# LiZhuoHong/SegLand

Hardware: AMD Instinct MI355X
Metric: 512x512 tiles/sec fwd+bwd PSPNet-POP (higher is better)
Workload: dtype bf16; 1 GPU; PSPNet-POP resnet50 bf16, batch 16/GPU, 512x512, 8 logit channels, train_base.py loop body (fwd+loss+bwd+clip+AdamW x2), 1 x MI355X; global_batch=16, parallelism=dp1

## Files before the change

include/segland_hip_debug.h:

```cpp
#ifndef SEGLAND_HIP_DEBUG_H
#define SEGLAND_HIP_DEBUG_H
#include "segland_hip.h"
#ifdef __cplusplus
extern "C" {
#endif

void sl_debug_reset(void);

void sl_debug_conv_affine(int on);
void sl_debug_conv_p9(int on);
void sl_debug_conv_p8_k1(int on);
void sl_debug_conv_ring192(int on);
void sl_debug_conv_ringn64(int on);
void sl_debug_conv_rows_small(int on);
void sl_debug_ppm_fact_walk(int on);
void sl_debug_conv_parity(int on);
void sl_debug_ring_small_k(int k);
void sl_debug_ring64_max_tiles(int tiles);
void sl_debug_wgrad3(int on);
void sl_debug_wgrad_bias(int on);
void sl_debug_wgrad_tr(int on);
void sl_debug_wgrad_pair_min(int rows);
void sl_debug_attn_valu(int v);

void sl_debug_p8_trace(void* buf);
void sl_debug_wgrad_trace(void* buf);
void sl_debug_wgrad3_trace(void* buf);
void sl_debug_attn_trace(void* buf);

int sl_debug_wgrad3_plan(const SlConvDesc* d, int* out);

#ifdef __cplusplus
}
#endif
#endif
```

segland_amd/csrc/api.cpp:

```cpp
#include <stdarg.h>
#include <stdio.h>
#include "common.h"

static thread_local char g_err[512] = "";

void sl_set_error(const char* fmt, ...) {
  va_list ap;
  va_start(ap, fmt);
  vsnprintf(g_err, sizeof(g_err), fmt, ap);
  va_end(ap);
}

extern "C" int sl_version(void) { return 100; }
extern "C" const char* sl_last_error_string(void) { return g_err; }
extern "C" int sl_hip_clear_error(void) { return (int)hipGetLastError(); }

#include "../../include/segland_hip_debug.h"
SlDebugState g_sl_debug;
extern "C" void sl_debug_reset(void) { g_sl_debug = SlDebugState(); }
extern "C" void sl_debug_conv_affine(int v) { g_sl_debug.conv_affine = v ? 1 : 0; }
extern "C" void sl_debug_conv_p9(int v) { g_sl_debug.conv_p9 = (v & 1) ? 1 : 0; }
extern "C" void sl_debug_conv_p8_k1(int v) { g_sl_debug.conv_p8_k1 = v ? 1 : 0; }
extern "C" void sl_debug_conv_ring192(int v) { g_sl_debug.conv_ring192 = v ? 1 : 0; }
extern "C" void sl_debug_conv_ringn64(int v) { g_sl_debug.conv_ringn64 = v ? 1 : 0; }
extern "C" void sl_debug_conv_rows_small(int v) { g_sl_debug.conv_rows_small = v ? 1 : 0; }
extern "C" void sl_debug_conv_parity(int v) { g_sl_debug.conv_parity = v ? 1 : 0; }
extern "C" void sl_debug_ppm_fact_walk(int v) { g_sl_debug.ppm_fact_walk = v ? 1 : 0; }
extern "C" void sl_debug_ring64_max_tiles(int v) { g_sl_debug.ring64_max_tiles = v; }
extern "C" void sl_debug_ring_small_k(int v) { g_sl_debug.ring_small_k = v; }
extern "C" void sl_debug_wgrad3(int v) { g_sl_debug.wgrad3 = v ? 1 : 0; }
extern "C" void sl_debug_wgrad_bias(int v) { g_sl_debug.wgrad_bias = v ? 1 : 0; }
extern "C" void sl_debug_wgrad_tr(int v) { g_sl_debug.wgrad_tr = v ? 1 : 0; }
extern "C" void sl_debug_wgrad_pair_min(int rows) { g_sl_debug.wgrad_pair_min_rows = rows; }
extern "C" void sl_debug_attn_valu(int v) { g_sl_debug.attn_valu = v; }
extern "C" void sl_debug_p8_trace(void* buf) { g_sl_debug.p8_trace = (unsigned long long*)buf; }
extern "C" void sl_debug_wgrad_trace(void* buf) { g_sl_debug.wgrad_trace = (unsigned long long*)buf; }
extern "C" void sl_debug_wgrad3_trace(void* buf) { g_sl_debug.wgrad3_trace = (unsigned long long*)buf; }
extern "C" void sl_debug_attn_trace(void* buf) { g_sl_debug.attn_trace = (unsigned long long*)buf; }
```

segland_amd/csrc/common.h:

```cpp
#pragma once
#include <hip/hip_runtime.h>
#include <stdint.h>
#include <stdio.h>
#include "../../include/segland_hip.h"

typedef unsigned short bf16_t;

typedef __attribute__((ext_vector_type(8))) __bf16 bf16x8_t;
typedef __attribute__((ext_vector_type(16))) float f32x16_t;
typedef __attribute__((ext_vector_type(4))) float f32x4_t;

__device__ __forceinline__ float bf2f(bf16_t v) { return __uint_as_float(((unsigned)v) << 16); }
__device__ __forceinline__ bf16_t f2bf(float f) {
  return __builtin_bit_cast(bf16_t, (__bf16)f);
}

template <typename T> __device__ __forceinline__ float to_f(T v);
template <> __device__ __forceinline__ float to_f<float>(float v) { return v; }
template <> __device__ __forceinline__ float to_f<bf16_t>(bf16_t v) { return bf2f(v); }
template <typename T> __device__ __forceinline__ T from_f(float v);
template <> __device__ __forceinline__ float from_f<float>(float v) { return v; }
template <> __device__ __forceinline__ bf16_t from_f<bf16_t>(float v) { return f2bf(v); }

template <typename T> struct Vec16 { static constexpr int N = 16 / sizeof(T); };

template <typename T> __device__ __forceinline__ void unpack16(const uint4& v, float* out);
template <> __device__ __forceinline__ void unpack16<float>(const uint4& v, float* out) {
  out[0] = __uint_as_float(v.x); out[1] = __uint_as_float(v.y); out[2] = __uint_as_float(v.z); out[3] = __uint_as_float(v.w);
}
template <> __device__ __forceinline__ void unpack16<bf16_t>(const uint4& v, float* out) {
  out[0] = __uint_as_float(v.x << 16); out[1] = __uint_as_float(v.x & 0xffff0000u);
  out[2] = __uint_as_float(v.y << 16); out[3] = __uint_as_float(v.y & 0xffff0000u);
  out[4] = __uint_as_float(v.z << 16); out[5] = __uint_as_float(v.z & 0xffff0000u);
  out[6] = __uint_as_float(v.w << 16); out[7] = __uint_as_float(v.w & 0xffff0000u);
}
template <typename T> __device__ __forceinline__ uint4 pack16(const float* in);
template <> __device__ __forceinline__ uint4 pack16<float>(const float* in) {
  return make_uint4(__float_as_uint(in[0]), __float_as_uint(in[1]), __float_as_uint(in[2]), __float_as_uint(in[3]));
}
template <> __device__ __forceinline__ uint4 pack16<bf16_t>(const float* in) {
  typedef __attribute__((ext_vector_type(2))) __bf16 bf16x2_t;
  typedef __attribute__((ext_vector_type(2))) float f32x2_t;
  uint4 r;
  r.x = __builtin_bit_cast(unsigned, __builtin_convertvector((f32x2_t){in[0], in[1]}, bf16x2_t));
  r.y = __builtin_bit_cast(unsigned, __builtin_convertvector((f32x2_t){in[2], in[3]}, bf16x2_t));
  r.z = __builtin_bit_cast(unsigned, __builtin_convertvector((f32x2_t){in[4], in[5]}, bf16x2_t));
  r.w = __builtin_bit_cast(unsigned, __builtin_convertvector((f32x2_t){in[6], in[7]}, bf16x2_t));
  return r;
}

__device__ __forceinline__ float sl_erf_as(float x) {
  const float ax = fabsf(x);
  const float t = __builtin_amdgcn_rcpf(fmaf(0.3275911f, ax, 1.f));
  float p = fmaf(1.061405429f, t, -1.453152027f);
  p = fmaf(p, t, 1.421413741f); p = fmaf(p, t, -0.284496736f); p = fmaf(p, t, 0.254829592f);
  const float r = fmaf(-p * t, __expf(-ax * ax), 1.f);
  return copysignf(r, x);
}
template <typename T> __device__ __forceinline__ float sl_gelu(float x) {
  if constexpr (sizeof(T) == 4) return 0.5f * x * (1.f + erff(x * 0.70710678118654752440f));
  else return 0.5f * x * (1.f + sl_erf_as(x * 0.70710678118654752440f));
}

template <typename T> __device__ __forceinline__ float sl_gelu_grad(float x) {
  const float pdf = 0.39894228040143267794f * __expf(-0.5f * x * x);
  float cdf;
  if constexpr (sizeof(T) == 4) cdf = 0.5f * (1.f + erff(x * 0.70710678118654752440f));
  else cdf = 0.5f * (1.f + sl_erf_as(x * 0.70710678118654752440f));
  return cdf + x * pdf;
}

__device__ __forceinline__ float wave_sum(float v) {
#pragma unroll
  for (int o = 32; o > 0; o >>= 1) v += __shfl_xor(v, o, 64);
  return v;
}

void sl_set_error(const char* fmt, ...);

struct SlDebugState {
  int conv_affine = 1;
  int conv_p9 = 1;
  int conv_p8_k1 = 1;
  int conv_ring192 = 1;
  int conv_ringn64 = 1;
  int conv_rows_small = 1;
  int ppm_fact_walk = 1;
  int conv_parity = 1;
  int ring_small_k = 128;
  long long ring64_max_tiles = 256;
  int wgrad3 = 1;
  int wgrad_bias = 1;
  int wgrad_tr = 1;
  long long wgrad_pair_min_rows = 0;
  int attn_valu = -1;
  unsigned long long* p8_trace = nullptr;
  unsigned long long* wgrad_trace = nullptr;
  unsigned long long* wgrad3_trace = nullptr;
  unsigned long long* attn_trace = nullptr;
};
extern SlDebugState g_sl_debug;
#define SL_REQUIRE(cond, ...)            \
  do {                                   \
    if (!(cond)) {                       \
      sl_set_error(__VA_ARGS__);         \
      return SL_EINVAL;                  \
    }                                    \
  } while (0)
#define SL_LAUNCH_CHECK(name)                                                \
  do {                                                                       \
    hipError_t e__ = hipGetLastError();                                      \
    if (e__ != hipSuccess) {                                                 \
      sl_set_error("%s: %s", name, hipGetErrorString(e__));                  \
      return (int)e__;                                                       \
    }                                                                        \
  } while (0)

__host__ __device__ static inline int cdiv(long long a, long long b) { return (int)((a + b - 1) / b); }

template <typename T>
__device__ __forceinline__ void sl_colsum_rows_block(const T* __restrict__ x, long long rows, int C, long long rows_per_block, float* __restrict__ part, int block, float* red) {
  constexpr int V = Vec16<T>::N;
  const int nvec = C / V;
  const int tpr = nvec < 256 ? nvec : 256, rpb = 256 / tpr;
  const int tr = threadIdx.x / tpr, tc = threadIdx.x % tpr;
  const long long r0 = (long long)block * rows_per_block, r1 = r0 + rows_per_block < rows ? r0 + rows_per_block : rows;
  for (int vc = tc; vc < nvec; vc += tpr) {
    float s[V];
#pragma unroll
    for (int k = 0; k < V; ++k) s[k] = 0.f;
    if (tr < rpb) {
      long long r = r0 + tr;
      for (; r + 3 * rpb < r1; r += 4 * rpb) {
        uint4 q[4];
#pragma unroll
        for (int u = 0; u < 4; ++u) q[u] = ((const uint4*)x)[(size_t)(r + u * rpb) * nvec + vc];
#pragma unroll
        for (int u = 0; u < 4; ++u) {
          float v[V];
          unpack16<T>(q[u], v);
#pragma unroll
          for (int k = 0; k < V; ++k) s[k] += v[k];
        }
      }
      for (; r < r1; r += rpb) {
        float v[V];
        unpack16<T>(((const uint4*)x)[(size_t)r * nvec + vc], v);
#pragma unroll
        for (int k = 0; k < V; ++k) s[k] += v[k];
      }
    }
    __syncthreads();
#pragma unroll
    for (int k = 0; k < V; ++k) red[threadIdx.x * V + k] = s[k];
    __syncthreads();
    if (tr == 0) {
#pragma unroll
      for (int k = 0; k < V; ++k) {
        float a = 0.f;
        for (int j = 0; j < rpb; ++j) a += red[(j * tpr + tc) * V + k];
        part[(size_t)block * C + vc * V + k] = a;
      }
    }
  }
}


inline long long sl_colsum_rows_chunk(long long rows, int C, int esize) {
  const int nvec = C * esize / 16, tpr = nvec < 256 ? nvec : 256, rpb = 256 / tpr;
  long long rpblk = (long long)rpb * 16;
  const long long cap = 2048;
  if ((rows + rpblk - 1) / rpblk > cap) rpblk = ((rows + cap - 1) / cap + rpb - 1) / rpb * rpb;
  return rpblk;
}
```

segland_amd/csrc/conv_gemm_common.h:

```cpp
#pragma once
#include <stdlib.h>
#include "common.h"

#ifndef SL_CH3_SPLIT
#define SL_CH3_SPLIT 2
#endif


struct ConvGemmParams {
  const void* src1; const void* src2;
  int C1, C2;
  const void* wt;
  void* out;
  int B, Hs, Ws;
  int Hd, Wd;
  int N, KH, KW, stride, pad, dil;
  int mode;
  const float* scale;
  const float* bias; int relu;
  const void* addend; const void* mask_src;
  const void* pre_addend;
  const unsigned char* addend_mask;
  float* stat_partial;
  const unsigned char* gate;
// ... 472 lines not shown
        for (int u = 0; u < CH; ++u) {
          const int m = mrow(it0 + u);
          if (m < p.M) prev[u] = *(const uint4*)((const T*)p.pre_addend + (size_t)m * p.N + ncol);
        }
      }
      unsigned abit[CH];
      if (p.addend) {
#pragma unroll
        for (int u = 0; u < CH; ++u) {
          const int m = mrow(it0 + u);
          if (m < p.M) addv[u] = *(const uint4*)((const T*)p.addend + (size_t)m * p.N + ncol);
        }
        if (p.addend_mask) {
#pragma unroll
          for (int u = 0; u < CH; ++u) {
            const int m = mrow(it0 + u);
            if (m < p.M) abit[u] = p.addend_mask[((size_t)m * p.N + ncol) / EPC];
          }
        }
      }
      if (p.mask_src) {
#pragma unroll
        for (int u = 0; u < CH; ++u) {
          const int m = mrow(it0 + u);
          if (m < p.M) mskv[u] = *(const uint4*)((const T*)p.mask_src + (size_t)m * p.N + ncol);
        }
      }
#pragma unroll
      for (int u = 0; u < CH; ++u) {
        const int row = r0 + (it0 + u) * RS;
        const int m = mrow(it0 + u);
        if (m < p.M) {
          float v[EPC];
          const uint4 raw = *(const uint4*)(smem + row * G::PITCH + cc * 16);
          unpack16<T>(raw, v);
          if (p.pre_addend) {
            float a[EPC];
            unpack16<T>(prev[u], a);
#pragma unroll
            for (int e = 0; e < EPC; ++e) v[e] += a[e];
          }
#pragma unroll
          for (int e = 0; e < EPC; ++e) { ssum[e] += v[e]; ssq[e] += v[e] * v[e]; }
          if (plain) { st16(out + (size_t)m * p.N + ncol, raw); continue; }
          if (p.bias || p.scale) {
#pragma unroll
            for (int e = 0; e < EPC; ++e) v[e] = v[e] * scl[e] + bias[e];
          }
          if (p.out2) {
            float g[EPC];
            unpack16<T>(pack16<T>(v), g);
#pragma unroll
            for (int e = 0; e < EPC; ++e) g[e] = sl_gelu<T>(g[e]);
            st16((T*)p.out2 + (size_t)m * p.N + ncol, pack16<T>(g));
          }
          if (p.row_scale) {
            const float rs = p.row_scale[m / (p.Hd * p.Wd)];
#pragma unroll
            for (int e = 0; e < EPC; ++e) v[e] *= rs;
          }
          if (p.addend) {
            float a[EPC];
            unpack16<T>(addv[u], a);
            if (p.addend_mask) {
              const unsigned bits = abit[u];
#pragma unroll
              for (int e = 0; e < EPC; ++e) a[e] = (bits >> e) & 1u ? a[e] : 0.f;
            }
#pragma unroll
            for (int e = 0; e < EPC; ++e) v[e] += a[e];
          }
          if (p.relu) {
#pragma unroll
            for (int e = 0; e < EPC; ++e) v[e] = v[e] > 0.f ? v[e] : 0.f;
          }
          if (p.mask_src) {
            float k[EPC];
            unpack16<T>(mskv[u], k);
            bool gelu = false;
            if constexpr (!SPLIT) gelu = (p.flags & 4) != 0;
            if (gelu) {
#pragma unroll
              for (int e = 0; e < EPC; ++e) v[e] *= sl_gelu_grad<T>(k[e]);
            } else {
#pragma unroll
              for (int e = 0; e < EPC; ++e) v[e] = k[e] > 0.f ? v[e] : 0.f;
            }
          }
          st16(out + (size_t)m * p.N + ncol, pack16<T>(v));
        }
      }
    }
    lds_barrier();
  }
  if (p.stat_partial) {
#pragma unroll
    for (int off = CPR; off < 64; off <<= 1) {
#pragma unroll
      for (int e = 0; e < EPC; ++e) { ssum[e] += __shfl_xor(ssum[e], off, 64); ssq[e] += __shfl_xor(ssq[e], off, 64); }
    }
    float* red = (float*)smem;
    const int wave = tid >> 6;
    if (lane < CPR) {
#pragma unroll
      for (int e = 0; e < EPC; ++e) {
        red[(wave * 2 + 0) * BN + cc * EPC + e] = ssum[e];
        red[(wave * 2 + 1) * BN + cc * EPC + e] = ssq[e];
      }
    }
    lds_barrier();
    for (int e = tid; e < 2 * BN; e += NT) {
      const int which = e / BN, col = e % BN;
      float t = 0.f;
#pragma unroll
      for (int w = 0; w < WM * WN; ++w) t += red[(w * 2 + which) * BN + col];
      p.stat_partial[((size_t)bm * 2 + which) * p.N + bn * BN + col] = t;
    }
  }
}

__device__ __attribute__((aligned(256))) unsigned char g_zero_page[256];

typedef __attribute__((address_space(3))) void lds_void_t;
typedef const __attribute__((address_space(1))) void gbl_void_t;

__device__ __forceinline__ void glds16(const void* g, unsigned char* l) {
  __builtin_amdgcn_global_load_lds((gbl_void_t*)g, (lds_void_t*)l, 16, 0, 0);
}

template <int RBYTES> __device__ __forceinline__ int ring_off(int row, int chunk);
template <> __device__ __forceinline__ int ring_off<128>(int row, int chunk) { return row * 128 + ((chunk ^ ((row >> 1) & 7)) << 4); }
template <> __device__ __forceinline__ int ring_off<64>(int row, int chunk) { return row * 64 + ((chunk ^ ((row >> 2) & 3)) << 4); }
template <int RBYTES> __device__ __forceinline__ int ring_swz(int row);
template <> __device__ __forceinline__ int ring_swz<128>(int row) { return (row >> 1) & 7; }
template <> __device__ __forceinline__ int ring_swz<64>(int row) { return (row >> 2) & 3; }

__device__ __forceinline__ void glds16_asm(const void* g, unsigned lds_addr) {
  unsigned keep;
  asm volatile("s_mov_b32 %0, m0\n\ts_mov_b32 m0, %2\n\ts_nop 0\n\tglobal_load_lds_dwordx4 %1, off\n\ts_mov_b32 m0, %0"
               : "=&s"(keep) : "v"(g), "s"(lds_addr) : "memory");
}
__device__ __forceinline__ void glds16x2_asm(const void* g0, const void* g1, unsigned lds_addr) {
  unsigned keep;
  asm volatile("s_mov_b32 %0, m0\n\ts_mov_b32 m0, %3\n\ts_nop 0\n\tglobal_load_lds_dwordx4 %1, off\n\ts_add_u32 m0, m0, 0x400\n\ts_nop 0\n\t"
               "global_load_lds_dwordx4 %2, off\n\ts_mov_b32 m0, %0"
               : "=&s"(keep) : "v"(g0), "v"(g1), "s"(lds_addr) : "memory", "scc");
}
__device__ __forceinline__ void glds16x2_sbase_asm(const void* sbase, unsigned off0, unsigned off1, unsigned lds_addr) {
  unsigned keep;
  asm volatile("s_mov_b32 %0, m0\n\ts_mov_b32 m0, %4\n\ts_nop 0\n\tglobal_load_lds_dwordx4 %2, %1\n\ts_add_u32 m0, m0, 0x400\n\ts_nop 0\n\t"
               "global_load_lds_dwordx4 %3, %1\n\ts_mov_b32 m0, %0"
               : "=&s"(keep) : "s"(sbase), "v"(off0), "v"(off1), "s"(lds_addr) : "memory", "scc");
}
__device__ __forceinline__ unsigned lds_addr_of(const unsigned char* p) {
  return (unsigned)(size_t)((const __attribute__((address_space(3))) unsigned char*)p);
}

template <int N> __device__ __forceinline__ void wait_vmcnt() { asm volatile("s_waitcnt vmcnt(%0)" ::"n"(N) : "memory"); }


}
```

segland_amd/csrc/conv_gemm_patch.hip:

```cpp
#include "conv_gemm_common.h"

namespace {

__device__ __forceinline__ void conv_store_partial(const ConvGemmParams& p, f32x16_t (&acc)[4][2], int part, int bm, int bn, int wm, int wn, int lane) {
  const int l31 = lane & 31, fh = lane >> 5;
  float* base = p.ws + (size_t)part * p.M * p.N + bn * 256 + wn * 32 + 4 * fh;
  int tbase = 0;
  if (p.tile16) { const int tx = p.Wd >> 4, ty = p.Hd >> 4; tbase = ((bm / (tx * ty)) * p.Hd + ((bm / tx) % ty) * 16) * p.Wd + (bm % tx) * 16; }
#pragma unroll
  for (int i = 0; i < 4; ++i) {
    const int R = (i >> 1) * 128 + wm * 64 + (i & 1) * 32 + l31;
    const int m = p.tile16 ? tbase + (R >> 4) * p.Wd + (R & 15) : bm * 256 + R;
    if (m < p.M) {
      float* row = base + (size_t)m * p.N;
#pragma unroll
      for (int j = 0; j < 2; ++j)
#pragma unroll
        for (int q = 0; q < 4; ++q)
          *(float4*)(row + j * 128 + 8 * q) = make_float4(acc[i][j][4 * q + 0], acc[i][j][4 * q + 1], acc[i][j][4 * q + 2], acc[i][j][4 * q + 3]);
    }
  }
}

template <typename T>
// ... 174 lines not shown

  int bm, bn;
  tile_of(blockIdx.x, bm, bn);
  setup(bm, bn);
  issue_first();
  int younger = 0;
  const bool counted = p.flags & 1;
#pragma unroll 1
  for (int tile = blockIdx.x; tile < ntiles; tile += gridDim.x) {
    f32x16_t acc[4][2];
#pragma unroll
    for (int i = 0; i < 4; ++i)
#pragma unroll
      for (int j = 0; j < 2; ++j)
#pragma unroll
        for (int r = 0; r < 16; ++r) acc[i][j][r] = 0.f;

    int tap2 = 0, ct2 = 0;
    adv(tap2, ct2);
    if (nk > 1) {
      issueB(0, tap2, ct2, p8_slot_b0(1)); issueA(0, tap2, ct2, p8_slot_a0(1)); issueA(1, tap2, ct2, p8_slot_a1(1)); issueB(1, tap2, ct2, p8_slot_b1(1));
      switch (younger) { case 16: wait_vmcnt<24>(); break; case 17: wait_vmcnt<25>(); break; case 32: wait_vmcnt<40>(); break; case 48: wait_vmcnt<56>(); break; case 49: wait_vmcnt<57>(); break; default: wait_vmcnt<8>(); }
    } else wait_vmcnt<0>();
    adv(tap2, ct2);
    __builtin_amdgcn_s_barrier();
    if (p.trace && tile == (int)blockIdx.x) tr1 = __builtin_amdgcn_s_memtime();
    uint4 a[4][2], b0k[4], b1k[4];
#pragma unroll
    for (int ks = 0; ks < 4; ++ks) { a[ks][0] = ldA(p8_slot_a0(0), 0, ks); a[ks][1] = ldA(p8_slot_a0(0), 1, ks); b0k[ks] = ldB(p8_slot_b0(0), ks); }

    int s3 = 0;
    if constexpr (!K1) {
    for (int i = 0; i < nk; ++i) {
      const int par = i & 1;
      const int s3n = s3 == 2 ? 0 : s3 + 1, s3nn = s3 == 0 ? 2 : s3 - 1;
      const int b0nxt = p8_slot_b0(s3n), b0nn = p8_slot_b0(s3nn);
      const int a1cur = p8_slot_a1(par), b1cur = p8_slot_b1(par), a0nxt = p8_slot_a0(s3n), a0nn = p8_slot_a0(s3nn);
      const bool more2 = i + 2 < nk;
#pragma unroll
      for (int q = 0; q < 16; ++q) {
        const int ph = q >> 2, ks = q & 3;
        const int ih = ph >> 1, jh = (ph == 1 || ph == 2) ? 1 : 0;
        if ((ks == 0 || ks == 2) && more2 && (ks == 2) == (wm == 1)) {
          if (ph == 0) issueB(0, tap2, ct2, b0nn);
          if (ph == 1) issueA(0, tap2, ct2, a0nn);
          if (ph == 3) { issueA(1, tap2, ct2, a1cur); issueB(1, tap2, ct2, b1cur); }
        }
        if (ph == 0) b1k[ks] = ldB(b1cur, ks);
        const uint4 bq = (ph == 0 || ph == 3) ? b0k[ks] : b1k[ks];
        Mma<T>::run(bq, a[ks][0], acc[ih * 2 + 0][jh]);
        Mma<T>::run(bq, a[ks][1], acc[ih * 2 + 1][jh]);
        if (ph == 1) { a[ks][0] = ldA(a1cur, 0, ks); a[ks][1] = ldA(a1cur, 1, ks); }
        if (ph == 3) { a[ks][0] = ldA(a0nxt, 0, ks); a[ks][1] = ldA(a0nxt, 1, ks); b0k[ks] = ldB(b0nxt, ks); }
        if (ks == 3) {
          if (ph == 2) { if (more2) wait_vmcnt<8>(); else if (i + 1 < nk) wait_vmcnt<4>(); else wait_vmcnt<0>(); }
          if (ph == 3) { if (more2) wait_vmcnt<8>(); else wait_vmcnt<0>(); }
          if (ph >= 2) __builtin_amdgcn_s_barrier();
        }
      }
      adv(tap2, ct2);
      s3 = s3 == 2 ? 0 : s3 + 1;
    }
    } else {
      auto ktile = [&](int i, auto tail_c) {
        constexpr int TAIL = decltype(tail_c)::value;
        const int par = i & 1;
        const int s3n = s3 == 2 ? 0 : s3 + 1, s3nn = s3 == 0 ? 2 : s3 - 1;
        const int b0nxt = p8_slot_b0(s3n), b0nn = p8_slot_b0(s3nn);
        const int a1cur = p8_slot_a1(par), b1cur = p8_slot_b1(par), a0nxt = p8_slot_a0(s3n), a0nn = p8_slot_a0(s3nn);
#pragma unroll
        for (int q = 0; q < 16; ++q) {
          const int ph = q >> 2, ks = q & 3;
          const int ih = ph >> 1, jh = (ph == 1 || ph == 2) ? 1 : 0;
          if (TAIL == 0 && (ks == 0 || ks == 2) && (ks == 2) == (wm == 1)) {
            if (ph == 0) issueB(0, 0, 0, b0nn);
            if (ph == 1) issueA(0, 0, 0, a0nn);
            if (ph == 3) { issueA(1, 0, 0, a1cur); issueB(1, 0, 0, b1cur); }
          }
          if (ph == 0) b1k[ks] = ldB(b1cur, ks);
          const uint4 bq = (ph == 0 || ph == 3) ? b0k[ks] : b1k[ks];
          Mma<T>::run(bq, a[ks][0], acc[ih * 2 + 0][jh]);
          Mma<T>::run(bq, a[ks][1], acc[ih * 2 + 1][jh]);
          if (ph == 1) { a[ks][0] = ldA(a1cur, 0, ks); a[ks][1] = ldA(a1cur, 1, ks); }
          if (ph == 3) { a[ks][0] = ldA(a0nxt, 0, ks); a[ks][1] = ldA(a0nxt, 1, ks); b0k[ks] = ldB(b0nxt, ks); }
          if (ks == 3) {
            if (ph == 2) wait_vmcnt<TAIL == 0 ? 8 : TAIL == 1 ? 4 : 0>();
            if (ph == 3) wait_vmcnt<TAIL == 0 ? 8 : 0>();
            if (ph >= 2) __builtin_amdgcn_s_barrier();
          }
        }
        s3 = s3 == 2 ? 0 : s3 + 1;
      };
      int i = 0;
#pragma unroll 1
      for (; i + 2 < nk; ++i) ktile(i, std::integral_constant<int, 0>());
      if (nk > 1) { ktile(i, std::integral_constant<int, 1>()); ++i; }
      ktile(i, std::integral_constant<int, 2>());
    }
    if (p.trace && tile == (int)blockIdx.x) tr2 = __builtin_amdgcn_s_memtime();
    lds_barrier();
    const int cbm = bm, cbn = bn;
    if (tile + (int)gridDim.x < ntiles) {
      tile_of(tile + gridDim.x, bm, bn);
      setup(bm, bn);
      issue_first();
    }
    younger = conv_epilogue_lds<T, BM, BN, 2, 4, true, GATE, AFF>(p, acc, cbm, cbn, wm, wn, lane, tid, smem);
    if (!counted) younger = 0;
    lds_barrier();
  }
  if (p.trace && tid == 0) {
    unsigned long long* t = p.trace + (size_t)blockIdx.x * 8;
    t[0] = tr0; t[1] = tr1; t[2] = tr2; t[3] = __builtin_amdgcn_s_memtime(); t[4] = __builtin_amdgcn_s_getreg((4 << 0) | (0 << 6) | (31 << 11)); t[5] = __builtin_amdgcn_s_getreg((20 << 0) | (0 << 6) | (31 << 11));
  }
}

int launch_splitk_finish(ConvGemmParams& p, hipStream_t st) {
  const size_t nvec = (size_t)p.M * p.N / 8;
  const int blocks = (int)((nvec + 255) / 256 < 4096 ? (nvec + 255) / 256 : 4096);
  hipLaunchKernelGGL(conv_splitk_finish_kernel<bf16_t>, dim3(blocks), dim3(256), 0, st, p);
  SL_LAUNCH_CHECK("conv_splitk_finish_kernel");
  return 0;
}

}

int slconv::launch_p8(ConvGemmParams& p, hipStream_t st) {
  p.gridM = cdiv(p.M, 256);
  p.gridN = p.N / 256;
  p.trace = g_sl_debug.p8_trace;
  p.flags |= 1;
  static bool attr_set = false;
  if (!attr_set) {
    const void* all[6] = {(const void*)conv_gemm_p8_kernel<0, false>, (const void*)conv_gemm_p8_kernel<1, false>, (const void*)conv_gemm_p8_kernel<2, false>,
                          (const void*)conv_gemm_p8_kernel<0, true>,  (const void*)conv_gemm_p8_kernel<1, true>,  (const void*)conv_gemm_p8_kernel<2, true>};
    for (const void* f : all) (void)hipFuncSetAttribute(f, hipFuncAttributeMaxDynamicSharedMemorySize, (int)P8_LDS);
    attr_set = true;
  }
  const int ntiles = p.gridM * p.gridN;
  const int epi = p.gate ? 1 : (p.bias || p.scale) && !p.stat_partial ? 2 : 0;
  const bool k1 = g_sl_debug.conv_p8_k1 && p.KH == 1 && p.KW == 1 && p.pad == 0 && p.C2 == 0 && !p.sub;
  void (*const kern[2][3])(ConvGemmParams) = {{conv_gemm_p8_kernel<0, false>, conv_gemm_p8_kernel<1, false>, conv_gemm_p8_kernel<2, false>},
                                              {conv_gemm_p8_kernel<0, true>, conv_gemm_p8_kernel<1, true>, conv_gemm_p8_kernel<2, true>}};
  hipLaunchKernelGGL(kern[k1][epi], dim3(ntiles > 256 ? 256 : ntiles), dim3(512), P8_LDS, st, p);
  SL_LAUNCH_CHECK("conv_gemm_p8_kernel");
  return 0;
}

namespace {
constexpr int P9_PATCH = 576 * 128;
constexpr int P9_LDS = P9_PATCH + 4 * P8_SLOT;
constexpr int P9_PATCH1 = 42 * 1024;
constexpr int P9_LDS1 = 2 * P9_PATCH1 + 4 * P8_SLOT;
template <int EPI>
__global__ __launch_bounds__(512) void conv_gemm_p9_kernel(ConvGemmParams p) {
  using T = bf16_t;
  constexpr int BM = 256, BN = 256;
  constexpr bool GATE = EPI == 1, SPLITK = EPI == 2;
  extern __shared__ __attribute__((aligned(16))) unsigned char smem[];
  const int tid = threadIdx.x, lane = tid & 63;
  const int wave = __builtin_amdgcn_readfirstlane(tid >> 6);
  const int wm = wave >> 2, wn = wave & 3;
  const int KS = SPLITK ? p.ksplit : 1;
  const int part = SPLITK ? (int)(blockIdx.x % KS) : 0;
  int bid = blockIdx.x / KS;
  {
    const int nwg = p.gridM * p.gridN, q = nwg >> 3, r = nwg & 7, xcd = bid & 7, idx = bid >> 3;
    bid = (xcd < r ? xcd * (q + 1) : r * (q + 1) + (xcd - r) * q) + idx;
  }
  const int GN = p.gridN > 2 && p.gridN % 2 == 0 && !(p.flags & 16) ? 2 : p.gridN;
  const int grp = bid / (p.gridM * GN), rem = bid - grp * (p.gridM * GN);
  const int bm = rem / GN, bn = grp * GN + rem % GN;
  const int d = p.dil, PW = 16 + 2 * d, PP = PW * PW;
  const int CT = p.C1;
  const int cbeg = SPLITK ? (CT / 64) * part / KS : 0, nchunk = SPLITK ? (CT / 64) * (part + 1) / KS : CT / 64;
  const int tx = p.Ws >> 4, ty = p.Hs >> 4;
  const int bx = bm % tx, by = (bm / tx) % ty, bb = bm / (tx * ty);
  const int y0 = by * 16 - d, x0 = bx * 16 - d;
  const unsigned lds_base = __builtin_amdgcn_readfirstlane(lds_addr_of(smem));
  const int lr = lane >> 3, lpos = lane & 7;
  const unsigned char* zsrc = g_zero_page + lpos * 16;

  constexpr int NPI = 9;
  const unsigned char* psrc[NPI];
#pragma unroll
  for (int j = 0; j < NPI; ++j) {
    const int pr = (j * 8 + wave) * 8 + lr;
    const int py = pr / PW, px = pr - py * PW;
    const int iy = y0 + py, ix = x0 + px;
    const bool ok = pr < PP && (unsigned)iy < (unsigned)p.Hs && (unsigned)ix < (unsigned)p.Ws;
    psrc[j] = ok ? (const unsigned char*)p.src1 + ((size_t)(bb * p.Hs + iy) * p.Ws + ix) * CT * sizeof(T) + ((lpos ^ ((px >> 1) & 7)) << 4) : nullptr;
  }
  const bool dbuf = d == 1 && !(p.flags & 8);
  const int boff = dbuf ? 2 * P9_PATCH1 : P9_PATCH;
  auto issue_patch = [&](int chunk) {
    const unsigned dst = lds_base + (dbuf && (chunk & 1) ? P9_PATCH1 : 0);
#pragma unroll
    for (int j = 0; j < NPI; ++j) {
      if ((j * 8 + wave) * 8 < PP)
        glds16_asm(psrc[j] ? psrc[j] + (size_t)chunk * 128 : zsrc, dst + (j * 8 + wave) * 1024);
    }
  };
  const size_t wpitch = (size_t)9 * CT * sizeof(T);
  int rsw[2];
  const unsigned char* wptr[2][2];
#pragma unroll
  for (int j = 0; j < 2; ++j) rsw[j] = (lpos ^ (((j * 8 + lr) >> 1) & 7)) * 16;
#pragma unroll
  for (int h = 0; h < 2; ++h)
#pragma unroll
    for (int j = 0; j < 2; ++j) wptr[h][j] = (const unsigned char*)p.wt + (size_t)(bn * BN + h * 128 + wave * 16 + j * 8 + lr) * wpitch + rsw[j];
  auto issueB = [&](int tap, int chunk, int par) {
    const size_t koff = ((size_t)tap * CT + chunk * 64) * sizeof(T);
#pragma unroll
    for (int h = 0; h < 2; ++h) {
      const unsigned dst = lds_base + boff + (par * 2 + h) * P8_SLOT + wave * 2048;
#pragma unroll
      for (int j = 0; j < 2; ++j) glds16_asm(wptr[h][j] + koff, dst + j * 1024);
    }
  };
  const int l31 = lane & 31, fh = lane >> 5;
  int foff[4];
#pragma unroll
  for (int ks = 0; ks < 4; ++ks) foff[ks] = l31 * 128 + (((2 * ks + fh) ^ ((l31 >> 1) & 7)) << 4);
  const unsigned char* fb = smem + boff + wn * (32 * 128);
  auto ldB = [&](int slot_off, int ks) { return *(const uint4*)(fb + slot_off + foff[ks]); };
  int prow[2][2];
#pragma unroll
  for (int h = 0; h < 2; ++h)
#pragma unroll
    for (int i2 = 0; i2 < 2; ++i2) prow[h][i2] = (h * 8 + wm * 4 + i2 * 2 + (l31 >> 4)) * PW + (l31 & 15);
  auto ldA = [&](int h, int i2, int toff, int ks, int pbase = 0) {
    const int pr = prow[h][i2] + (toff >> 8);
    const int px = (l31 & 15) + (toff & 255);
    return *(const uint4*)(smem + pbase + pr * 128 + (((2 * ks + fh) ^ ((px >> 1) & 7)) << 4));
  };

  f32x16_t acc[4][2];
#pragma unroll
  for (int i = 0; i < 4; ++i)
#pragma unroll
    for (int j = 0; j < 2; ++j)
#pragma unroll
      for (int r = 0; r < 16; ++r) acc[i][j][r] = 0.f;

  const int NK = 9 * (nchunk - cbeg);
  auto toff_of = [&](int tap) { const int t2 = p.mode ? 8 - tap : tap; return ((((t2 / 3) * PW + (t2 % 3)) * d) << 8) | ((t2 % 3) * d); };
  issue_patch(cbeg);
  issueB(0, cbeg, 0);
  issueB(1, cbeg, 1);
  wait_vmcnt<0>();
  __builtin_amdgcn_s_barrier();
  uint4 a[4][2], b0k[4], b1k[4];
  {
    const int toff = toff_of(0), pb0 = dbuf && (cbeg & 1) ? P9_PATCH1 : 0;
#pragma unroll
    for (int ks = 0; ks < 4; ++ks) { a[ks][0] = ldA(0, 0, toff, ks, pb0); a[ks][1] = ldA(0, 1, toff, ks, pb0); b0k[ks] = ldB(0, ks); }
  }
  int tap = 0, chunk = cbeg;
#pragma unroll 1
  for (int k = 0; k < NK; ++k) {
    const int par = k & 1;
    const int b1s = (par * 2 + 1) * P8_SLOT, b0n = ((par ^ 1) * 2 + 0) * P8_SLOT;
    const int toff = toff_of(tap);
    const bool last_tap = tap == 8;
    const int toffn = toff_of(last_tap ? 0 : tap + 1);
    const int pb = dbuf && (chunk & 1) ? P9_PATCH1 : 0, pbn = dbuf && last_tap ? (pb ? 0 : P9_PATCH1) : pb;
#pragma unroll
    for (int q = 0; q < 16; ++q) {
      const int ph = q >> 2, ks = q & 3;
      const int ih = ph >> 1, jh = (ph == 1 || ph == 2) ? 1 : 0;
      if (ph == 0) b1k[ks] = ldB(b1s, ks);
      const uint4 bq = (ph == 0 || ph == 3) ? b0k[ks] : b1k[ks];
      Mma<T>::run(bq, a[ks][0], acc[ih * 2 + 0][jh]);
      Mma<T>::run(bq, a[ks][1], acc[ih * 2 + 1][jh]);
      if (ph == 1) { a[ks][0] = ldA(1, 0, toff, ks, pb); a[ks][1] = ldA(1, 1, toff, ks, pb); }
      if (ph == 2 && ks == 3) {
        wait_vmcnt<0>();
        __builtin_amdgcn_s_barrier();
        if (dbuf && tap == 0 && chunk + 1 < nchunk) issue_patch(chunk + 1);
        if (k + 2 < NK) {
          int t2 = tap + 2, c2 = chunk;
          if (t2 >= 9) { t2 -= 9; ++c2; }
          issueB(t2, c2, par);
        }
      }
      if (ph == 3) {
        b0k[ks] = ldB(b0n, ks);
        if (!last_tap || dbuf) { a[ks][0] = ldA(0, 0, toffn, ks, pbn); a[ks][1] = ldA(0, 1, toffn, ks, pbn); }
      }
    }
    if (last_tap) {
      tap = 0; ++chunk;
      if (chunk < nchunk && !dbuf) {
        __builtin_amdgcn_s_barrier();
        issue_patch(chunk);
        wait_vmcnt<0>();
        __builtin_amdgcn_s_barrier();
#pragma unroll
        for (int ks = 0; ks < 4; ++ks) { a[ks][0] = ldA(0, 0, toffn, ks); a[ks][1] = ldA(0, 1, toffn, ks); }
      }
    } else ++tap;
  }
  if constexpr (SPLITK) { conv_store_partial(p, acc, part, bm, bn, wm, wn, lane); return; }
  lds_barrier();
  conv_epilogue_lds<T, BM, BN, 2, 4, true, GATE>(p, acc, bm, bn, wm, wn, lane, tid, smem);
}

}

bool slconv::p9_on() { return g_sl_debug.conv_p9 != 0; }
bool slconv::p9_shape(const ConvGemmParams& p) {
  return p9_on() && p.KH == 3 && p.KW == 3 && p.stride == 1 && p.pad == p.dil && (p.dil == 1 || p.dil == 2 || p.dil == 4) && p.C2 == 0 && p.C1 % 64 == 0 && p.N % 256 == 0 &&
         p.Hs == p.Hd && p.Ws == p.Wd && p.Hs % 16 == 0 && p.Ws % 16 == 0 && ((long long)p.M >= 32768 || p.ksplit > 1) &&
         !(p.out2 || p.row_scale);
}
int slconv::launch_p9(ConvGemmParams& p, hipStream_t st) {
  p.gridM = p.M / 256; p.gridN = p.N / 256; p.tile16 = 1;
  static bool attr_set = false;
  if (!attr_set) {
    (void)hipFuncSetAttribute((const void*)conv_gemm_p9_kernel<0>, hipFuncAttributeMaxDynamicSharedMemorySize, (int)(P9_LDS1 > P9_LDS ? P9_LDS1 : P9_LDS));
    (void)hipFuncSetAttribute((const void*)conv_gemm_p9_kernel<1>, hipFuncAttributeMaxDynamicSharedMemorySize, (int)(P9_LDS1 > P9_LDS ? P9_LDS1 : P9_LDS));
    (void)hipFuncSetAttribute((const void*)conv_gemm_p9_kernel<2>, hipFuncAttributeMaxDynamicSharedMemorySize, (int)(P9_LDS1 > P9_LDS ? P9_LDS1 : P9_LDS));
    attr_set = true;
  }
  if (p.ksplit > 1) {
    hipLaunchKernelGGL(conv_gemm_p9_kernel<2>, dim3(p.gridM * p.gridN * p.ksplit), dim3(512), p.dil == 1 ? P9_LDS1 : P9_LDS, st, p);
    SL_LAUNCH_CHECK("conv_gemm_p9_kernel (split-K)");
    return launch_splitk_finish(p, st);
  }
  if (p.gate) hipLaunchKernelGGL(conv_gemm_p9_kernel<1>, dim3(p.gridM * p.gridN), dim3(512), p.dil == 1 ? P9_LDS1 : P9_LDS, st, p);
  else        hipLaunchKernelGGL(conv_gemm_p9_kernel<0>, dim3(p.gridM * p.gridN), dim3(512), p.dil == 1 ? P9_LDS1 : P9_LDS, st, p);
  SL_LAUNCH_CHECK("conv_gemm_p9_kernel");
  return 0;
}
```

Before: 692.3 tiles/s.

## Add lean dilation-specialized p9 conv kernel with compile-time tap offsets

Adds a templated variant of the 3x3 patch conv GEMM kernel, specialized on dilation and flip. Patch and weight tap offsets become compile-time immediates in precomputed LDS addresses, and all nine taps are fully unrolled. Global-to-LDS loads are batched into multi-issue asm helpers that step m0. The goal is to cut per-tap address arithmetic, VGPR pressure and instruction overhead in the main MFMA loop, at the cost of more kernel instantiations and larger code.

After: 707.1 tiles/s (median of 6 runs). 2.1% higher.

```diff
diff --git a/include/segland_hip_debug.h b/include/segland_hip_debug.h
--- a/include/segland_hip_debug.h
+++ b/include/segland_hip_debug.h
@@ -9,6 +9,7 @@
 
 void sl_debug_conv_affine(int on);
 void sl_debug_conv_p9(int on);
+void sl_debug_conv_p9_lean(int on);
 void sl_debug_conv_p8_k1(int on);
 void sl_debug_conv_ring192(int on);
 void sl_debug_conv_ringn64(int on);
diff --git a/segland_amd/csrc/api.cpp b/segland_amd/csrc/api.cpp
--- a/segland_amd/csrc/api.cpp
+++ b/segland_amd/csrc/api.cpp
@@ -20,6 +20,7 @@
 extern "C" void sl_debug_reset(void) { g_sl_debug = SlDebugState(); }
 extern "C" void sl_debug_conv_affine(int v) { g_sl_debug.conv_affine = v ? 1 : 0; }
 extern "C" void sl_debug_conv_p9(int v) { g_sl_debug.conv_p9 = (v & 1) ? 1 : 0; }
+extern "C" void sl_debug_conv_p9_lean(int v) { g_sl_debug.conv_p9_lean = v ? 1 : 0; }
 extern "C" void sl_debug_conv_p8_k1(int v) { g_sl_debug.conv_p8_k1 = v ? 1 : 0; }
 extern "C" void sl_debug_conv_ring192(int v) { g_sl_debug.conv_ring192 = v ? 1 : 0; }
 extern "C" void sl_debug_conv_ringn64(int v) { g_sl_debug.conv_ringn64 = v ? 1 : 0; }
diff --git a/segland_amd/csrc/common.h b/segland_amd/csrc/common.h
--- a/segland_amd/csrc/common.h
+++ b/segland_amd/csrc/common.h
@@ -81,6 +81,7 @@
 struct SlDebugState {
   int conv_affine = 1;
   int conv_p9 = 1;
+  int conv_p9_lean = 1;
   int conv_p8_k1 = 1;
   int conv_ring192 = 1;
   int conv_ringn64 = 1;
diff --git a/segland_amd/csrc/conv_gemm_common.h b/segland_amd/csrc/conv_gemm_common.h
--- a/segland_amd/csrc/conv_gemm_common.h
+++ b/segland_amd/csrc/conv_gemm_common.h
@@ -648,6 +648,19 @@
                "global_load_lds_dwordx4 %3, %1\n\ts_mov_b32 m0, %0"
                : "=&s"(keep) : "s"(sbase), "v"(off0), "v"(off1), "s"(lds_addr) : "memory", "scc");
 }
+__device__ __forceinline__ void glds16x4_sbase_asm(const void* sbase, unsigned off0, unsigned off1, unsigned off2, unsigned off3, unsigned lds_addr) {
+  unsigned keep;
+  asm volatile("s_mov_b32 %0, m0\n\ts_mov_b32 m0, %6\n\ts_nop 0\n\tglobal_load_lds_dwordx4 %2, %1\n\ts_add_u32 m0, m0, 0x400\n\ts_nop 0\n\t"
+               "global_load_lds_dwordx4 %3, %1\n\ts_add_u32 m0, m0, 0x3c00\n\ts_nop 0\n\tglobal_load_lds_dwordx4 %4, %1\n\ts_add_u32 m0, m0, 0x400\n\ts_nop 0\n\t"
+               "global_load_lds_dwordx4 %5, %1\n\ts_mov_b32 m0, %0"
+               : "=&s"(keep) : "s"(sbase), "v"(off0), "v"(off1), "v"(off2), "v"(off3), "s"(lds_addr) : "memory", "scc");
+}
+template <int STEP> __device__ __forceinline__ void glds16x2_step_asm(const void* g0, const void* g1, unsigned lds_addr) {
+  unsigned keep;
+  asm volatile("s_mov_b32 %0, m0\n\ts_mov_b32 m0, %3\n\ts_nop 0\n\tglobal_load_lds_dwordx4 %1, off\n\ts_add_u32 m0, m0, %4\n\ts_nop 0\n\t"
+               "global_load_lds_dwordx4 %2, off\n\ts_mov_b32 m0, %0"
+               : "=&s"(keep) : "v"(g0), "v"(g1), "s"(lds_addr), "n"(STEP) : "memory", "scc");
+}
 __device__ __forceinline__ unsigned lds_addr_of(const unsigned char* p) {
   return (unsigned)(size_t)((const __attribute__((address_space(3))) unsigned char*)p);
 }
diff --git a/segland_amd/csrc/conv_gemm_patch.hip b/segland_amd/csrc/conv_gemm_patch.hip
--- a/segland_amd/csrc/conv_gemm_patch.hip
+++ b/segland_amd/csrc/conv_gemm_patch.hip
@@ -350,7 +350,14 @@
 constexpr int P9_LDS = P9_PATCH + 4 * P8_SLOT;
 constexpr int P9_PATCH1 = 42 * 1024;
 constexpr int P9_LDS1 = 2 * P9_PATCH1 + 4 * P8_SLOT;
-template <int EPI>
+typedef unsigned u32x4_t __attribute__((ext_vector_type(4)));
+__device__ __forceinline__ uint4 lds_read16(unsigned addr) {
+  const u32x4_t v = *(const __attribute__((address_space(3))) u32x4_t*)(size_t)addr;
+  return make_uint4(v.x, v.y, v.z, v.w);
+}
+template <int I> using p9_int = std::integral_constant<int, I>;
+
+template <int EPI, int D, bool FLIP>
 __global__ __launch_bounds__(512) void conv_gemm_p9_kernel(ConvGemmParams p) {
   using T = bf16_t;
   constexpr int BM = 256, BN = 256;
@@ -369,7 +376,7 @@
   const int GN = p.gridN > 2 && p.gridN % 2 == 0 && !(p.flags & 16) ? 2 : p.gridN;
   const int grp = bid / (p.gridM * GN), rem = bid - grp * (p.gridM * GN);
   const int bm = rem / GN, bn = grp * GN + rem % GN;
-  const int d = p.dil, PW = 16 + 2 * d, PP = PW * PW;
+  const int d = D ? D : p.dil, PW = 16 + 2 * d, PP = PW * PW;
   const int CT = p.C1;
   const int cbeg = SPLITK ? (CT / 64) * part / KS : 0, nchunk = SPLITK ? (CT / 64) * (part + 1) / KS : CT / 64;
   const int tx = p.Ws >> 4, ty = p.Hs >> 4;
@@ -378,6 +385,8 @@
   const unsigned lds_base = __builtin_amdgcn_readfirstlane(lds_addr_of(smem));
   const int lr = lane >> 3, lpos = lane & 7;
   const unsigned char* zsrc = g_zero_page + lpos * 16;
+  f32x16_t acc[4][2];
+  if constexpr (D == 0) {
 
   constexpr int NPI = 9;
   const unsigned char* psrc[NPI];
@@ -434,7 +443,6 @@
     return *(const uint4*)(smem + pbase + pr * 128 + (((2 * ks + fh) ^ ((px >> 1) & 7)) << 4));
   };
 
-  f32x16_t acc[4][2];
 #pragma unroll
   for (int i = 0; i < 4; ++i)
 #pragma unroll
@@ -500,6 +508,140 @@
       }
     } else ++tap;
   }
+
+  } else {
+    constexpr int LPW = 16 + 2 * D, LPP = LPW * LPW;
+    constexpr int NPI = 9;
+    constexpr bool DBUF = D == 1;
+    constexpr int BOFF = DBUF ? 2 * P9_PATCH1 : P9_PATCH;
+    static_assert(((10 * LPW + (2 * LPW + 2) * D) * 128) < 65536, "ds_read immediates");
+    const unsigned char* pptr[10]; unsigned okm = 0;
+#pragma unroll
+    for (int j = 0; j < NPI; ++j) {
+      const int pr = (j * 8 + wave) * 8 + lr;
+      const int py = pr / LPW, px = pr - py * LPW;
+      const int iy = y0 + py, ix = x0 + px;
+      const bool ok = pr < LPP && (unsigned)iy < (unsigned)p.Hs && (unsigned)ix < (unsigned)p.Ws;
+      pptr[j] = ok ? (const unsigned char*)p.src1 + (((size_t)(bb * p.Hs + iy) * p.Ws + ix) * CT + (size_t)cbeg * 64) * sizeof(T) + ((lpos ^ ((px >> 1) & 7)) << 4) : zsrc;
+      okm |= ok ? 1u << j : 0u;
+    }
+    pptr[9] = zsrc;
+    auto issue_patch = [&](unsigned buf) {
+      const unsigned dst = lds_base + buf + wave * 1024;
+#pragma unroll
+      for (int j = 0; j < 10; j += 2) {
+        const bool all0 = (j * 8 + 7) * 8 < LPP, all1 = ((j + 1) * 8 + 7) * 8 < LPP;
+        if (all0 && all1) glds16x2_step_asm<8192>(pptr[j], pptr[j + 1], dst + j * 8192);
+        else {
+          if (all0 || (j * 64 < LPP && (j * 8 + wave) * 8 < LPP)) glds16_asm(pptr[j], dst + j * 8192);
+          if (all1 || ((j + 1) * 64 < LPP && ((j + 1) * 8 + wave) * 8 < LPP)) glds16_asm(pptr[j + 1], dst + (j + 1) * 8192);
+        }
+      }
+#pragma unroll
+      for (int j = 0; j < NPI; ++j)
+        if (j * 64 < LPP) pptr[j] += ((okm >> j) & 1u) << 7;
+    };
+    const unsigned wpitch = 9u * CT * (unsigned)sizeof(T);
+    unsigned woff[4];
+#pragma unroll
+    for (int h = 0; h < 2; ++h)
+#pragma unroll
+      for (int j = 0; j < 2; ++j) woff[h * 2 + j] = (unsigned)(h * 128 + j * 8 + lr) * wpitch + ((lpos ^ (((j * 8 + lr) >> 1) & 7)) * 16);
+    const unsigned char* wcur = (const unsigned char*)p.wt + (size_t)(bn * BN + wave * 16) * wpitch + (size_t)cbeg * 128;
+    const long long tapstep = (long long)CT * (long long)sizeof(T), wrapstep = 128 - 8 * tapstep;
+    unsigned bd[2];
+    bd[0] = lds_base + BOFF + wave * 2048; bd[1] = bd[0] + 2 * P8_SLOT;
+    const int l31 = lane & 31, fh = lane >> 5;
+    unsigned pcur = DBUF && (cbeg & 1) ? P9_PATCH1 : 0;
+    unsigned ab[3][4], fbs[2][4];
+#pragma unroll
+    for (int kx = 0; kx < 3; ++kx)
+#pragma unroll
+      for (int ks = 0; ks < 4; ++ks)
+        ab[kx][ks] = lds_base + pcur + ((wm * 4 + (l31 >> 4)) * LPW + (l31 & 15)) * 128 + (((2 * ks + fh) ^ ((((l31 & 15) + kx * D) >> 1) & 7)) << 4);
+#pragma unroll
+    for (int ks = 0; ks < 4; ++ks) {
+      fbs[0][ks] = lds_base + BOFF + wn * (32 * 128) + l31 * 128 + (((2 * ks + fh) ^ ((l31 >> 1) & 7)) << 4);
+      fbs[1][ks] = fbs[0][ks] + 2 * P8_SLOT;
+    }
+#pragma unroll
+    for (int i = 0; i < 4; ++i)
+#pragma unroll
+      for (int j = 0; j < 2; ++j)
+#pragma unroll
+        for (int r = 0; r < 16; ++r) acc[i][j][r] = 0.f;
+
+    issue_patch(pcur);
+    glds16x4_sbase_asm(wcur, woff[0], woff[1], woff[2], woff[3], bd[0]); wcur += tapstep;
+    glds16x4_sbase_asm(wcur, woff[0], woff[1], woff[2], woff[3], bd[1]); wcur += tapstep;
+    wait_vmcnt<0>();
+    __builtin_amdgcn_s_barrier();
+    constexpr int T0 = FLIP ? 8 : 0, KX0 = T0 % 3, OFF0 = ((T0 / 3) * LPW + KX0) * D * 128;
+    uint4 a[4][2], b0k[4], b1k[4];
+#pragma unroll
+    for (int ks = 0; ks < 4; ++ks) { a[ks][0] = lds_read16(ab[KX0][ks] + OFF0); a[ks][1] = lds_read16(ab[KX0][ks] + OFF0 + 2 * LPW * 128); b0k[ks] = lds_read16(fbs[0][ks]); }
+
+    auto ktile = [&](auto tc, auto lc) {
+      constexpr int t = decltype(tc)::value; constexpr bool LAST = decltype(lc)::value;
+      constexpr int sp = t & 1;
+      constexpr int tw = FLIP ? 8 - t : t, tn = t == 8 ? 0 : t + 1, twn = FLIP ? 8 - tn : tn;
+      constexpr int kx = tw % 3, kxn = twn % 3;
+      constexpr int off = ((tw / 3) * LPW + kx) * D * 128, offn = ((twn / 3) * LPW + kxn) * D * 128;
+#pragma unroll
+      for (int q = 0; q < 16; ++q) {
+        const int ph = q >> 2, ks = q & 3;
+        const int ih = ph >> 1, jh = (ph == 1 || ph == 2) ? 1 : 0;
+        if (ph == 0) b1k[ks] = lds_read16(fbs[sp][ks] + P8_SLOT);
+        const uint4 bq = (ph == 0 || ph == 3) ? b0k[ks] : b1k[ks];
+        Mma<T>::run(bq, a[ks][0], acc[ih * 2 + 0][jh]);
+        Mma<T>::run(bq, a[ks][1], acc[ih * 2 + 1][jh]);
+        if (ph == 1) { a[ks][0] = lds_read16(ab[kx][ks] + off + 8 * LPW * 128); a[ks][1] = lds_read16(ab[kx][ks] + off + 10 * LPW * 128); }
+        if (ph == 2 && ks == 3) {
+          wait_vmcnt<0>();
+          __builtin_amdgcn_s_barrier();
+          if (DBUF && t == 0 && !LAST) issue_patch(P9_PATCH1 - pcur);
+          if (!(LAST && t >= 7)) { glds16x4_sbase_asm(wcur, woff[0], woff[1], woff[2], woff[3], bd[sp]); wcur += t == 6 ? wrapstep : tapstep; }
+          if (DBUF && t == 8 && !LAST) {
+            const unsigned nxt = P9_PATCH1 - pcur, delta = nxt - pcur;
+#pragma unroll
+            for (int x = 0; x < 3; ++x)
+#pragma unroll
+              for (int y = 0; y < 4; ++y) ab[x][y] += delta;
+            pcur = nxt;
+          }
+        }
+        if (ph == 3 && !(LAST && t == 8)) {
+          b0k[ks] = lds_read16(fbs[sp ^ 1][ks]);
+          if (t < 8 || DBUF) { a[ks][0] = lds_read16(ab[kxn][ks] + offn); a[ks][1] = lds_read16(ab[kxn][ks] + offn + 2 * LPW * 128); }
+        }
+      }
+    };
+    auto chunk_body = [&](auto lc) {
+      constexpr bool LAST = decltype(lc)::value;
+#pragma unroll
+      for (int x = 0; x < 3; ++x)
+#pragma unroll
+        for (int y = 0; y < 4; ++y) asm volatile("" : "+v"(ab[x][y]));
+      ktile(p9_int<0>(), lc); ktile(p9_int<1>(), lc); ktile(p9_int<2>(), lc); ktile(p9_int<3>(), lc); ktile(p9_int<4>(), lc);
+      ktile(p9_int<5>(), lc); ktile(p9_int<6>(), lc); ktile(p9_int<7>(), lc); ktile(p9_int<8>(), lc);
+      if constexpr (!LAST) {
+#pragma unroll
+        for (int ks = 0; ks < 4; ++ks) { const unsigned x = fbs[0][ks]; fbs[0][ks] = fbs[1][ks]; fbs[1][ks] = x; }
+        { const unsigned x = bd[0]; bd[0] = bd[1]; bd[1] = x; }
+        if constexpr (!DBUF) {
+          __builtin_amdgcn_s_barrier();
+          issue_patch(0);
+          wait_vmcnt<0>();
+          __builtin_amdgcn_s_barrier();
+#pragma unroll
+          for (int ks = 0; ks < 4; ++ks) { a[ks][0] = lds_read16(ab[KX0][ks] + OFF0); a[ks][1] = lds_read16(ab[KX0][ks] + OFF0 + 2 * LPW * 128); }
+        }
+      }
+    };
+#pragma unroll 1
+    for (int chunk = cbeg; chunk + 1 < nchunk; ++chunk) chunk_body(std::false_type());
+    chunk_body(std::true_type());
+  }
   if constexpr (SPLITK) { conv_store_partial(p, acc, part, bm, bn, wm, wn, lane); return; }
   lds_barrier();
   conv_epilogue_lds<T, BM, BN, 2, 4, true, GATE>(p, acc, bm, bn, wm, wn, lane, tid, smem);
@@ -515,20 +657,27 @@
 }
 int slconv::launch_p9(ConvGemmParams& p, hipStream_t st) {
   p.gridM = p.M / 256; p.gridN = p.N / 256; p.tile16 = 1;
+  typedef void (*kern_t)(ConvGemmParams);
+#define P9_ROW(E, F) {{conv_gemm_p9_kernel<E, 0, false>, conv_gemm_p9_kernel<E, 0, false>}, {conv_gemm_p9_kernel<E, 1, false>, conv_gemm_p9_kernel<E, 1, F>}, \
+                      {conv_gemm_p9_kernel<E, 2, false>, conv_gemm_p9_kernel<E, 2, F>}, {conv_gemm_p9_kernel<E, 4, false>, conv_gemm_p9_kernel<E, 4, F>}}
+  static const kern_t kern[3][4][2] = {P9_ROW(0, true), P9_ROW(1, true), P9_ROW(2, false)};
+#undef P9_ROW
   static bool attr_set = false;
   if (!attr_set) {
-    (void)hipFuncSetAttribute((const void*)conv_gemm_p9_kernel<0>, hipFuncAttributeMaxDynamicSharedMemorySize, (int)(P9_LDS1 > P9_LDS ? P9_LDS1 : P9_LDS));
-    (void)hipFuncSetAttribute((const void*)conv_gemm_p9_kernel<1>, hipFuncAttributeMaxDynamicSharedMemorySize, (int)(P9_LDS1 > P9_LDS ? P9_LDS1 : P9_LDS));
-    (void)hipFuncSetAttribute((const void*)conv_gemm_p9_kernel<2>, hipFuncAttributeMaxDynamicSharedMemorySize, (int)(P9_LDS1 > P9_LDS ? P9_LDS1 : P9_LDS));
+    for (int e = 0; e < 3; ++e)
+      for (int v = 0; v < 4; ++v)
+        for (int f = 0; f < 2; ++f) (void)hipFuncSetAttribute((const void*)kern[e][v][f], hipFuncAttributeMaxDynamicSharedMemorySize, (int)(P9_LDS1 > P9_LDS ? P9_LDS1 : P9_LDS));
     attr_set = true;
   }
+  const bool lean = g_sl_debug.conv_p9_lean && !(p.flags & 8) && (p.ksplit <= 1 || (p.mode == 0 && p.ksplit <= p.C1 / 64));
+  const int v = !lean ? 0 : p.dil == 1 ? 1 : p.dil == 2 ? 2 : 3, f = lean && p.mode != 0;
+  const size_t lds = p.dil == 1 ? P9_LDS1 : P9_LDS;
   if (p.ksplit > 1) {
-    hipLaunchKernelGGL(conv_gemm_p9_kernel<2>, dim3(p.gridM * p.gridN * p.ksplit), dim3(512), p.dil == 1 ? P9_LDS1 : P9_LDS, st, p);
+    hipLaunchKernelGGL(kern[2][v][f], dim3(p.gridM * p.gridN * p.ksplit), dim3(512), lds, st, p);
     SL_LAUNCH_CHECK("conv_gemm_p9_kernel (split-K)");
     return launch_splitk_finish(p, st);
   }
-  if (p.gate) hipLaunchKernelGGL(conv_gemm_p9_kernel<1>, dim3(p.gridM * p.gridN), dim3(512), p.dil == 1 ? P9_LDS1 : P9_LDS, st, p);
-  else        hipLaunchKernelGGL(conv_gemm_p9_kernel<0>, dim3(p.gridM * p.gridN), dim3(512), p.dil == 1 ? P9_LDS1 : P9_LDS, st, p);
+  hipLaunchKernelGGL(kern[p.gate ? 1 : 0][v][f], dim3(p.gridM * p.gridN), dim3(512), lds, st, p);
   SL_LAUNCH_CHECK("conv_gemm_p9_kernel");
   return 0;
 }
```
